# jgsimard/big-dreamer

Hardware: AMD Instinct MI355X
Metric: latent transitions/sec (RSSM + imagination) at batch=50 chunk=50 H=15 (higher is better)
Workload: dtype f32

## Files before the change

### big_dreamer_amd/csrc/observe_cluster.hip

```cpp
#include "bd_cluster.h"

namespace bd {

#ifdef BD_STAMPS
__device__ unsigned long long g_cstamps[64];
#define BD_CSTAMP(slot)                                                                                  \
    do {                                                                                                 \
        if (blockIdx.x == 0 && threadIdx.x == 0 && t == 5) g_cstamps[slot] = __builtin_amdgcn_s_memtime(); \
    } while (0)
#else
#define BD_CSTAMP(slot)
#endif

__global__ __launch_bounds__(kThreads) void observe_cfwd_kernel(bd_observe_fwd_args a_, float* __restrict__ ws, int C,
                                                                int tiles, unsigned spin_limit) {
    extern __shared__ __attribute__((aligned(16))) float smem[];
    BD_KARGS(bd_observe_fwd_args, ap);
#define a (*ap)
    const ScanDims d(a.Be, a.S, a.A, a.Hd);
    const int tile = blockIdx.x / C, c = blockIdx.x - tile * C;
    const int row0 = tile * 16;
    const int F = a.Be + a.S;
    const int nh = d.Kb_h * kFragFloats;
    const int Nb = d.Kb_h;
// ... 394 lines not shown
                    const floatx4* __restrict__ Whz = reinterpret_cast<const floatx4*>(a.wt_hz) + off;
                    const floatx4* __restrict__ Whn = reinterpret_cast<const floatx4*>(a.wt_hn) + off;
                    for (int kb = wave; kb < d.Kb_h; kb += kWaves) {
                        const floatx4 ar = R4[kb * 64], az = Z4[kb * 64], ai = I4[kb * 64], ah = H4[kb * 64];
                        const floatx4 bir = Wir[kb * 64], biz = Wiz[kb * 64], bin = Win[kb * 64];
                        const floatx4 bhr = Whr[kb * 64], bhz = Whz[kb * 64], bhn = Whn[kb * 64];
#pragma unroll
                        for (int j = 0; j < 4; ++j) {
                            DX = mfma16(ar[j], bir[j], DX);
                            DH = mfma16(ar[j], bhr[j], DH);
                            DX = mfma16(az[j], biz[j], DX);
                            DH = mfma16(az[j], bhz[j], DH);
                            DX = mfma16(ai[j], bin[j], DX);
                            DH = mfma16(ah[j], bhn[j], DH);
                        }
                    }
                    floatx4* g = G4 + ((wave * kLocalBlocks + bi) * 2) * 64 + lane;
                    g[0] = DX; g[64] = DH;
                }
            }
        }
        lds_barrier();
        float de_keep[4] = {0.f, 0.f, 0.f, 0.f};
        if (reducer) {
            floatx4 DX = floatx4{0.f, 0.f, 0.f, 0.f}, DH = DX;
            for (int w = 0; w < kWaves; ++w) {
                const floatx4* g = G4 + ((w * kLocalBlocks + wave) * 2) * 64 + lane;
                DX += g[0]; DH += g[64];
            }
            const int col = my_nb * 16 + (lane & 15);
            float* xb = xbuf + (size_t)(epoch & 1) * X.bwd_copy;
#pragma unroll
            for (int r = 0; r < 4; ++r) {
                const int grow = row0 + 4 * (lane >> 4) + r;
                const int off = acc_frag_off(my_nb, lane, r);
                float de = 0.f, carry = 0.f;
                if (grow < a.B && col < a.Be) {
                    de = DX[r] * elu_grad_from_out(svx[r]);
                    carry = dhc[off] + DH[r];
                }
                st_sc1(xb + off, carry);
                st_sc1(xb + nh + off, de);
                de_keep[r] = de;
            }
        }
        BD_CSTAMP(20);
        publish(flags + c, epoch);
        if (reducer) {
            const int col = my_nb * 16 + (lane & 15);
#pragma unroll
            for (int r = 0; r < 4; ++r) {
                const int grow = row0 + 4 * (lane >> 4) + r;
                if (grow < a.B && col < a.Be) a.d_embed_pre[(tb + grow) * a.Be + col] = de_keep[r];
            }
        }
        BD_CSTAMP(21);
        wait_all(flags, C, epoch, err, spin_limit, kErrBwd);
        BD_CSTAMP(22);
        gather_payload(xbuf + (size_t)(epoch & 1) * X.bwd_copy, dhc, 2 * nh);
        lds_barrier();
        BD_KARGS_FRESH(ap);
        BD_CSTAMP(23);
        tile_linear<1>(dE, d.Kb_h, a.wt_embed_s, nullptr, a.S, [&](int, int nb, floatx4 acc) {
            const int col = nb * 16 + (lane & 15);
#pragma unroll
            for (int r = 0; r < 4; ++r) {
                const int row = 4 * (lane >> 4) + r, grow = row0 + row;
                if (col < a.S) {
                    float v = 0.f;
                    if (grow < a.B) v = acc[r] * (a.nonterm ? a.nonterm[tb + grow] : 1.f);
                    ds_plain[row * a.S + col] = v;
                }
            }
        }, scratch);
        lds_barrier();
        BD_CSTAMP(24);
    }
#undef a
}

static int pick_cluster(int B, int Be) {
    const int Nb = cdiv(Be, 16), tiles = cdiv(B, 16);
    int C = tiles * Nb <= 256 ? Nb : cdiv(Nb, kLocalBlocks);
    if (C < 1) C = 1;
    return (C <= kMaxCluster && tiles * C <= 256) ? C : 0;
}

unsigned& cluster_spin_limit() {
    static unsigned v = kSpinLimit;
    return v;
}

}

extern "C" {
using namespace bd;

#ifdef BD_STAMPS
int bd_debug_cstamps(unsigned long long* out64) {
    return hipMemcpyFromSymbol(out64, HIP_SYMBOL(g_cstamps), sizeof(unsigned long long) * 64) == hipSuccess ? 0 : -1;
}
#endif

int bd_observe_cluster_size(int B, int Be) { return pick_cluster(B, Be); }

size_t bd_observe_cluster_ws_floats(int B, int Be) {
    const int tiles = cdiv(B, 16);
    size_t per_tile = ObsClusterWs(cdiv(Be, 16)).per_tile;
    const int C = pick_cluster(B, Be);
    if (C > 0 && kKsCopies * KsBuf(C).total > per_tile) per_tile = kKsCopies * KsBuf(C).total;
    return cluster_ws_header_floats(tiles) + (size_t)tiles * per_tile;
}

size_t bd_observe_cluster_err_offset(int B) { return cluster_ws_flag_floats(cdiv(B, 16)); }

size_t bd_scan_lds_bytes(int kernel, int Be, int S, int D, int C, int A, int Hd, int Cm) {
    const bool cat = kernel >= BD_SCAN_OBSERVE_CAT_FWD && kernel <= BD_SCAN_OBSERVE_CAT_CBWD;
    const bool catc = kernel == BD_SCAN_OBSERVE_CAT_CFWD || kernel == BD_SCAN_OBSERVE_CAT_CBWD;
    if (kernel < BD_SCAN_OBSERVE_FWD || kernel > BD_SCAN_OBSERVE_CAT_CBWD) return fail("bd_scan_lds_bytes: unknown kernel %d", kernel), 0;
    if (Be <= 0 || A <= 0 || Hd <= 0 || (cat ? (D <= 0 || C <= 0) : S <= 0)) return fail("bd_scan_lds_bytes: bad dims"), 0;
    if (catc && (Cm <= 0 || D % Cm != 0)) return fail("bd_scan_lds_bytes: cluster size %d does not divide D=%d", Cm, D), 0;
    const ScanDims d(Be, cat ? 0 : S, A, Hd);
    const int nfm = catc ? D / Cm : D, nbl = nfm * C / 16;
    int total = 0;
    bool ok = false;
#define BD_LAYOUT(id, ...)            \
    case id: {                        \
        const __VA_ARGS__;            \
        total = L.total;              \
        ok = L.vec_ok();              \
    } break
    switch (kernel) {
        BD_LAYOUT(BD_SCAN_OBSERVE_FWD, ObserveFwdLds L(d, S, kObsFwdScratch));
        BD_LAYOUT(BD_SCAN_OBSERVE_BWD, ObserveBwdLds L(d, S, kObsBwdScratch));
        BD_LAYOUT(BD_SCAN_OBSERVE_CFWD, ObserveFwdLds L(d, S, kObsCfwdScratch));
        BD_LAYOUT(BD_SCAN_OBSERVE_CBWD, ObserveBwdLds L(d, S, kObsCbwdScratch));
        BD_LAYOUT(BD_SCAN_OBSERVE_KFWD, KsplitFwdLds L(d, S));
        BD_LAYOUT(BD_SCAN_OBSERVE_KBWD, KsplitBwdLds L(d, S));
        BD_LAYOUT(BD_SCAN_IMAGINE_FWD, ImagineFwdLds L(d, A));
        BD_LAYOUT(BD_SCAN_IMAGINE_BWD, ImagineBwdLds L(d, S));
        BD_LAYOUT(BD_SCAN_OBSERVE_CAT_FWD, CatObserveFwdLds L(d, Be, D, CatFull(D, C), 0));
        BD_LAYOUT(BD_SCAN_OBSERVE_CAT_BWD, CatObserveBwdLds L(d, CatGeo(D, C), 0));
        BD_LAYOUT(BD_SCAN_IMAGINE_CAT_FWD, CatImagineFwdLds L(d, Be, Hd, D, A, CatFull(D, C)));
        BD_LAYOUT(BD_SCAN_IMAGINE_CAT_BWD, CatImagineBwdLds L(d, CatGeo(D, C)));
        BD_LAYOUT(BD_SCAN_OBSERVE_CAT_CFWD, CatObserveFwdLds L(d, Be, D, CatFull(nfm, C), cat_cluster_scratch(nbl, true)));
        BD_LAYOUT(BD_SCAN_OBSERVE_CAT_CBWD, CatObserveBwdLds L(d, CatGeo(nfm, C), cat_cluster_scratch(nbl, false)));
    }
#undef BD_LAYOUT
    if (!ok) return fail("bd_scan_lds_bytes: kernel %d: misaligned LDS layout", kernel), 0;
    return (size_t)total * sizeof(float);
}

int bd_observe_cluster_set_ksplit(int mode) {
    if (mode != -1 && mode != 0) return fail("bd_observe_cluster_set_ksplit: mode %d (expected -1 or 0)", mode);
    ksplit_mode() = mode;
    return 0;
}

int bd_observe_cluster_set_spin_limit(unsigned limit) {
    cluster_spin_limit() = limit ? limit : kSpinLimit;
    return 0;
}

int bd_observe_cluster_status(float* ws, int B, void* stream) {
    unsigned* w = reinterpret_cast<unsigned*>(ws) + bd_observe_cluster_err_offset(B);
    unsigned e = 0;
    if (hipMemcpyAsync(&e, w, sizeof(e), hipMemcpyDeviceToHost, (hipStream_t)stream) != hipSuccess ||
        hipStreamSynchronize((hipStream_t)stream) != hipSuccess)
        return fail("bd_observe_cluster_status: copy failed");
    if (e == 0) return 0;
    if (hipMemsetAsync(w, 0, sizeof(e), (hipStream_t)stream) != hipSuccess) return fail("bd_observe_cluster_status: clear failed");
    return fail("bd_observe_cluster_status: a cluster member timed out waiting for its peers (%s%s scan): results of that "
                "launch are wrong", (e & kErrFwd) ? "forward" : "", (e & kErrBwd) ? ((e & kErrFwd) ? "+backward" : "backward") : "");
}

int bd_observe_forward_cluster(const bd_observe_fwd_args* a, float* ws, size_t ws_floats, void* stream) {
    BD_REQUIRE(a && ws && a->T > 0 && a->B > 0 && a->Be > 0 && a->S > 0 && a->A > 0 && a->Hd > 0,
               "bd_observe_forward_cluster: bad arguments");
    BD_REQUIRE(a->w_embed_s && a->w_embed_a && a->b_embed && a->w_ir && a->w_iz && a->w_in && a->w_hr && a->w_hz &&
                   a->w_hn && a->b_ih && a->b_hh && a->w_q1h && a->b_q1 && a->w_q2m && a->w_q2s && a->b_q2 &&
                   a->init_belief && a->init_state && a->actions && a->pre_emb && a->eps_post && a->feat &&
                   a->post_mean && a->post_std, "bd_observe_forward_cluster: missing pointers");
    BD_REQUIRE(a->S <= kHeadMaxN, "bd_observe_forward_cluster: state width above %d", kHeadMaxN);
    const int C = pick_cluster(a->B, a->Be);
    BD_REQUIRE(C > 0, "bd_observe_forward_cluster: B=%d, Be=%d do not fit the cluster variant", a->B, a->Be);
    const int tiles = cdiv(a->B, 16);
    BD_REQUIRE(ws_floats >= bd_observe_cluster_ws_floats(a->B, a->Be), "bd_observe_forward_cluster: workspace too small");
    const ScanDims d(a->Be, a->S, a->A, a->Hd);
    const ObserveFwdLds L(d, a->S, kObsCfwdScratch);
    BD_REQUIRE(L.vec_ok(), "bd_observe_forward_cluster: misaligned LDS layout");
    const size_t lds = (size_t)L.total * sizeof(float);
    BD_REQUIRE(lds <= (size_t)kMaxLds, "bd_observe_forward_cluster: needs %zu B of LDS", lds);
    if (ksplit_ok(a->Be, a->S, a->A, a->Hd, C))
        return launch_observe_kfwd(a, ws, C, tiles, (hipStream_t)stream);
    if (allow_big_lds(observe_cfwd_kernel)) return -1;
    const size_t dyn = launch_lds(observe_cfwd_kernel, lds, "bd_observe_forward_cluster");
    if (!dyn) return -1;
    if (hipMemsetAsync(ws, 0, cluster_ws_flag_floats(tiles) * sizeof(float), (hipStream_t)stream) != hipSuccess)
        return fail("bd_observe_forward_cluster: memset failed");
    hipLaunchKernelGGL(observe_cfwd_kernel, dim3(tiles * C), dim3(kThreads), dyn, (hipStream_t)stream, *a, ws, C, tiles,
                       cluster_spin_limit());
    BD_CHECK_LAUNCH("bd_observe_forward_cluster");
    return 0;
}

int bd_observe_backward_cluster(const bd_observe_bwd_args* a, float* ws, size_t ws_floats, void* stream) {
    BD_REQUIRE(a && ws && a->T > 0 && a->B > 0 && a->Be > 0 && a->S > 0 && a->A > 0 && a->Hd > 0,
               "bd_observe_backward_cluster: bad arguments");
    BD_REQUIRE(a->wt_embed_s && a->wt_ir && a->wt_iz && a->wt_in && a->wt_hr && a->wt_hz && a->wt_hn && a->wt_q1h &&
                   a->wt_q2m && a->wt_q2s && a->init_belief && a->eps_post && a->feat && a->post_std && a->sv_x &&
                   a->sv_gates && a->sv_q && a->dfeat && a->d_embed_pre && a->d_gi && a->d_gh && a->d_q1_pre && a->d_q2_out,
               "bd_observe_backward_cluster: missing pointers");
    const int C = pick_cluster(a->B, a->Be);
    BD_REQUIRE(C > 0, "bd_observe_backward_cluster: B=%d, Be=%d do not fit the cluster variant", a->B, a->Be);
    const int tiles = cdiv(a->B, 16);
    BD_REQUIRE(ws_floats >= bd_observe_cluster_ws_floats(a->B, a->Be), "bd_observe_backward_cluster: workspace too small");
    const ScanDims d(a->Be, a->S, a->A, a->Hd);
    const ObserveBwdLds L(d, a->S, kObsCbwdScratch);
    BD_REQUIRE(L.vec_ok(), "bd_observe_backward_cluster: misaligned LDS layout");
    const size_t lds = (size_t)L.total * sizeof(float);
    BD_REQUIRE(lds <= (size_t)kMaxLds, "bd_observe_backward_cluster: needs %zu B of LDS", lds);
    if (ksplit_ok(a->Be, a->S, a->A, a->Hd, C)) return launch_observe_kbwd(a, ws, C, tiles, (hipStream_t)stream);
    if (allow_big_lds(observe_cbwd_kernel)) return -1;
    const size_t dyn = launch_lds(observe_cbwd_kernel, lds, "bd_observe_backward_cluster");
    if (!dyn) return -1;
    if (hipMemsetAsync(ws, 0, cluster_ws_flag_floats(tiles) * sizeof(float), (hipStream_t)stream) != hipSuccess)
        return fail("bd_observe_backward_cluster: memset failed");
    hipLaunchKernelGGL(observe_cbwd_kernel, dim3(tiles * C), dim3(kThreads), dyn, (hipStream_t)stream, *a, ws, C, tiles,
                       cluster_spin_limit());
    BD_CHECK_LAUNCH("bd_observe_backward_cluster");
    return 0;
}

}
```

### big_dreamer_amd/csrc/observe_ksplit.hip

```cpp
#include "bd_cluster.h"

namespace bd {

#ifdef BD_STAMPS
__device__ unsigned long long g_kstamps[64];
#define BD_KSTAMP(slot)                                                                                  \
    do {                                                                                                 \
        if (blockIdx.x == 0 && threadIdx.x == 0 && t == 5) g_kstamps[slot] = __builtin_amdgcn_s_memtime(); \
    } while (0)
#else
#define BD_KSTAMP(slot)
#endif

constexpr int kKsMaxS = 4;
constexpr int kKsMaxA = 2;

__device__ __forceinline__ void ks_store4(float* p, floatx4 v) {
    asm volatile("s_nop 7\n\ts_nop 3\n\tglobal_store_dwordx4 %0, %1, off sc1\n\ts_nop 1" ::"v"(p), "v"(v) : "memory");
}
__device__ __forceinline__ floatx4 ks_load4(const float* p) {
    const unsigned long long lo = ld_sc1_u64(p), hi = ld_sc1_u64(p + 2);
    return floatx4{__uint_as_float((unsigned)lo), __uint_as_float((unsigned)(lo >> 32)), __uint_as_float((unsigned)hi),
                   __uint_as_float((unsigned)(hi >> 32))};
}
// ... 195 lines not shown
        float* hx = xb + kb_.g;
        BD_KSTAMP(0);
        BD_KARGS_FRESH(ap);
        BD_KSTAMP(1);
        {
            const floatx4* __restrict__ S4 = reinterpret_cast<const floatx4*>(sf) + lane;
            const floatx4* __restrict__ A4 = reinterpret_cast<const floatx4*>(af) + lane;
#pragma unroll
            for (int i = 0; i < 2; ++i) {
                const int nbo = wave + kWaves * i;
                if (nbo < Kb_h) {
                    floatx4 acc = be4x[i];
#pragma unroll
                    for (int kb = 0; kb < kKsMaxS; ++kb)
                        if (kb < Kb_s) acc = mfmaT(we_s[i][kb], S4[kb * 64], acc);
#pragma unroll
                    for (int kb = 0; kb < kKsMaxA; ++kb)
                        if (kb < Kb_a) acc = mfmaT(we_a[i][kb], A4[kb * 64], acc);
                    floatx4 x4;
                    const int col0 = nbo * 16 + 4 * (lane >> 4);
#pragma unroll
                    for (int j = 0; j < 4; ++j) x4[j] = (rok && col0 + j < a.Be) ? elu(acc[j]) : 0.f;
                    XF4[nbo * 64 + lane] = x4;
                    if (nbo == c && rok && a.sv_x) ks_put4(a.sv_x + (tb + grow) * a.Be + fcol0, x4, nbe);
                }
            }
        }
        lds_barrier();
        BD_KSTAMP(2);
        BD_KARGS_FRESH(ap);
        {
            floatx4 R = z4, Z = z4, NI = z4, NH = z4;
#pragma unroll
            for (int i = 0; i < 2; ++i) {
                const int kb = wave + kWaves * i;
                if (kb < Kb_h) {
                    const floatx4 xk = XF4[kb * 64 + lane], hk = HF4[kb * 64 + lane];
                    R = mfmaT(wg[i][0], xk, R); Z = mfmaT(wg[i][1], xk, Z); NI = mfmaT(wg[i][2], xk, NI);
                    R = mfmaT(wg[i][3], hk, R); Z = mfmaT(wg[i][4], hk, Z); NH = mfmaT(wg[i][5], hk, NH);
                }
            }
            GP4[(wave * 4 + 0) * 64 + lane] = R; GP4[(wave * 4 + 1) * 64 + lane] = Z;
            GP4[(wave * 4 + 2) * 64 + lane] = NI; GP4[(wave * 4 + 3) * 64 + lane] = NH;
        }
        lds_barrier();
        BD_KSTAMP(3);
        BD_KSTAMP(4);
        {
            const int g = wave & 3, half = wave >> 2;
            floatx4 s4 = z4;
#pragma unroll
            for (int w = 0; w < 4; ++w) s4 += GP4[((half * 4 + w) * 4 + g) * 64 + lane];
            RED4[wave * 64 + lane] = s4;
        }
        lds_barrier();
        {
            const floatx4 R = RED4[0 * 64 + lane] + RED4[4 * 64 + lane] + br4, Z = RED4[1 * 64 + lane] + RED4[5 * 64 + lane] + bz4;
            const floatx4 NI = RED4[2 * 64 + lane] + RED4[6 * 64 + lane] + bni4, NH = RED4[3 * 64 + lane] + RED4[7 * 64 + lane] + bnh4;
            floatx4 rr4, zz4, nn4;
#pragma unroll
            for (int i = 0; i < 4; ++i) {
                rr4[i] = sigmoidf(R[i]);
                zz4[i] = sigmoidf(Z[i]);
                nn4[i] = tanh_act(NI[i] + rr4[i] * NH[i]);
                h4[i] = (rok && i < nbe) ? (1.f - zz4[i]) * nn4[i] + zz4[i] * h4[i] : 0.f;
            }
            if (wave == 0) {
                ks_store4(hx + (size_t)c * 256 + lane * 4, h4);
                if (rok) {
                    ks_put4(a.feat + (tb + grow) * F + fcol0, h4, nbe);
                    if (a.sv_gates) {
                        float* gg = a.sv_gates + (tb + grow) * 4 * a.Be + fcol0;
                        ks_put4(gg, rr4, nbe); ks_put4(gg + a.Be, zz4, nbe); ks_put4(gg + 2 * a.Be, nn4, nbe); ks_put4(gg + 3 * a.Be, NH, nbe);
                    }
                }
            }
        }
        BD_KSTAMP(5);
        BD_KARGS_FRESH(ap);
        const float n_nt = load_nt(t + 1, tid), n_ac = load_ac(t + 1, tid);
        const floatx4 pre4 = rok ? ks_row4(a.pre_emb + (tb + grow) * a.Hd + fcol0, nhd) : z4;
        float eps = 0.f;
        {
            const int row = tid / a.S, col = tid - row * a.S;
            if (tid < 16 * a.S && row0 + row < a.B) eps = a.eps_post[(tb + row0 + row) * a.S + col];
        }
#pragma unroll
        for (int i = 0; i < 2; ++i) {
            const int nbo = wave + kWaves * i;
            if (nbo < Kb_hd) ks_emit(xb + kb_.q + (size_t)(nbo * C + c) * kKsImg, lane, mfmaT(wq[i], h4, z4));
        }
        BD_KSTAMP(6);
        ks_handoff(flags, c, C, (unsigned)(3 * t + 2), err, spin_limit, kErrFwd);
        BD_KSTAMP(7);
        REDB[wave * 64 + lane] = c < Kb_hd ? ks_reduce(xb + kb_.q + (size_t)(c * C) * kKsImg, kKsImg, wave, kWaves, C, lane) : z4;
#pragma unroll
        for (int i = 0; i < 2; ++i) {
            const int nbo = wave + kWaves * i;
            if (nbo < Kb_h) HF4[nbo * 64 + lane] = ks_load4(hx + (size_t)nbo * 256 + lane * 4);
        }
        lds_barrier();
        floatx4 q4 = bq4 + pre4;
        for (int w = 0; w < kWaves; ++w) q4 += REDB[w * 64 + lane];
#pragma unroll
        for (int i = 0; i < 4; ++i) q4[i] = (rok && i < nhd) ? elu(q4[i]) : 0.f;
        if (wave == 0 && rok && a.sv_q) ks_put4(a.sv_q + (tb + grow) * a.Hd + fcol0, q4, nhd);
        BD_KSTAMP(8);
        BD_KARGS_FRESH(ap);
        if (has_pair) ks_emit(xb + kb_.s + (size_t)(c * 8 + pair) * kKsImg, lane, mfmaT(wh, q4, z4));
        BD_KSTAMP(9);
        ks_handoff(flags, c, C, (unsigned)(3 * t + 3), err, spin_limit, kErrFwd);
        BD_KSTAMP(10);
        BD_KARGS_FRESH(ap);
        if (sums_pair) {
            floatx4 v = ks_reduce(xb + kb_.s + (size_t)pair * kKsImg, (size_t)8 * kKsImg, part, nparts, C, lane);
            if (part == 0) v += bh4;
            float* pl = plain + (size_t)part * 2 * 16 * Np;
#pragma unroll
            for (int i = 0; i < 4; ++i) pl[pair_raw * 16 * Np + frow * Np + pair_nb * 16 + 4 * (lane >> 4) + i] = v[i];
        }
        lds_barrier();
        if (tid < 16 * a.S) {
            const int e = tid;
            const int row = e / a.S, col = e - row * a.S;
            const int gr = row0 + row;
            float st = 0.f;
            if (gr < a.B) {
                float Mn = plain[row * Np + col], Rw = plain[16 * Np + row * Np + col];
                for (int pt = 1; pt < nparts; ++pt) {
                    Mn += plain[pt * 2 * 16 * Np + row * Np + col];
                    Rw += plain[pt * 2 * 16 * Np + 16 * Np + row * Np + col];
                }
                const float ee = eps;
                const float sd = softplusf(Rw) + a.min_std;
                st = Mn + sd * ee;
                if (lead) {
                    const size_t ix = (tb + gr) * a.S + col;
                    a.post_mean[ix] = Mn;
                    a.post_std[ix] = sd;
                    a.feat[(tb + gr) * F + a.Be + col] = st;
                }
            }
            const float mv = st * n_nt;
            sf[frag_idx(row, col)] = mv;
            if (lead && a.sv_s && t + 1 < a.T && gr < a.B) a.sv_s[(tb + a.B + gr) * a.S + col] = mv;
        }
        if (tid < 16 * Kb_a * 16) af[frag_idx(tid / (Kb_a * 16), tid % (Kb_a * 16))] = n_ac;
        lds_barrier();
        BD_KSTAMP(11);
    }
#undef a
}

__global__ __launch_bounds__(kThreads) void observe_kbwd_kernel(bd_observe_bwd_args a_, float* __restrict__ ws, int C, int tiles,
                                                                unsigned spin_limit) {
    extern __shared__ __attribute__((aligned(16))) float smem[];
    BD_KARGS(bd_observe_bwd_args, ap);
#define a (*ap)
    const ScanDims d(a.Be, a.S, a.A, a.Hd);
    const int Kb_h = d.Kb_h, Kb_s = d.Kb_s, Kb_hd = d.Kb_hd;
    const int tile = blockIdx.x / C, c = blockIdx.x - tile * C;
    const int row0 = tile * 16, F = a.Be + a.S;
    const int lane = threadIdx.x & 63;
    const int wave = __builtin_amdgcn_readfirstlane((int)(threadIdx.x >> 6));
    const KsplitBwdLds L(d, a.S);
    float* dM = smem + L.dM;
    float* dRaw = smem + L.dRaw;
    float* ds_plain = smem + L.ds_plain;
    const int nparts = L.nparts;
    const int dsp_stride = L.dsp_stride;
    float* red = smem + L.red;

    unsigned* flags = reinterpret_cast<unsigned*>(ws) + tile * kMaxCluster;
    unsigned* err = reinterpret_cast<unsigned*>(ws) + tiles * kMaxCluster;
    const KsBuf kb_(C);
    float* xbase = ws + cluster_ws_header_floats(tiles) + (size_t)tile * kKsCopies * kb_.total;

    floatx4 w2m[kKsMaxS], w2s[kKsMaxS];
#pragma unroll
    for (int kb = 0; kb < kKsMaxS; ++kb) {
        w2m[kb] = ks_frag(a.wt_q2m, c, Kb_s, kb, lane, kb < Kb_s && c < Kb_hd);
        w2s[kb] = ks_frag(a.wt_q2s, c, Kb_s, kb, lane, kb < Kb_s && c < Kb_hd);
    }
    floatx4 w1[2], wg[2][6];
#pragma unroll
    for (int i = 0; i < 2; ++i) {
        const int nbo = wave + kWaves * i;
        const bool ok = nbo < Kb_h;
        w1[i] = ks_frag(a.wt_q1h, nbo, Kb_hd, c, lane, ok && c < Kb_hd);
        wg[i][0] = ks_frag(a.wt_ir, nbo, Kb_h, c, lane, ok); wg[i][1] = ks_frag(a.wt_iz, nbo, Kb_h, c, lane, ok);
        wg[i][2] = ks_frag(a.wt_in, nbo, Kb_h, c, lane, ok); wg[i][3] = ks_frag(a.wt_hr, nbo, Kb_h, c, lane, ok);
        wg[i][4] = ks_frag(a.wt_hz, nbo, Kb_h, c, lane, ok); wg[i][5] = ks_frag(a.wt_hn, nbo, Kb_h, c, lane, ok);
    }
    const int sblk = wave % Kb_s, spart = wave / Kb_s;
    floatx4 wes = ks_frag(a.wt_embed_s, sblk, Kb_h, c, lane, spart == 0);
    const int frow = lane & 15, fcol0 = c * 16 + 4 * (lane >> 4);
    const int grow = row0 + frow;
    const int nbe = a.Be - fcol0 < 0 ? 0 : (a.Be - fcol0 < 4 ? a.Be - fcol0 : 4);
    const int nhd = a.Hd - fcol0 < 0 ? 0 : (a.Hd - fcol0 < 4 ? a.Hd - fcol0 : 4);
    const bool rok = grow < a.B;

    for (int i = threadIdx.x; i < nparts * dsp_stride; i += blockDim.x) ds_plain[i] = 0.f;
    lds_barrier();

    KS_SETTLE_BEGIN();
    ks_settle(w2m); ks_settle(w2s); ks_settle(w1); ks_settle(wg[0]); ks_settle(wg[1]);
    ks_settle(wes);
    const bool lead = (c == 0);
    floatx4* __restrict__ RED4 = reinterpret_cast<floatx4*>(red);
    floatx4* __restrict__ REDB = RED4 + kWaves * 64;
    const floatx4 z4 = floatx4{0.f, 0.f, 0.f, 0.f};
    floatx4 dhc4 = z4;
    unsigned epoch = 0;

    struct B1v { float dfs, dpm, eps, dps, pstd; };
    struct Svv { floatx4 svq4, svx4, gr4, gz4, gn4, gh4, hp4, dft4; };
    auto load_b1 = [&](int t, int i) {
        B1v v{0.f, 0.f, 0.f, 0.f, 0.f};
        const int r = i / (Kb_s * 16), k = i - r * (Kb_s * 16);
        const int gr = row0 + r;
        if (i < 16 * Kb_s * 16 && gr < a.B && k < a.S) {
            const size_t tb = (size_t)t * a.B, idx = (tb + gr) * a.S + k;
            v.dfs = a.dfeat[(tb + gr) * F + a.Be + k];
            v.dpm = a.dpost_mean ? a.dpost_mean[idx] : 0.f;
            v.eps = a.eps_post[idx];
            v.dps = a.dpost_std ? a.dpost_std[idx] : 0.f;
            v.pstd = a.post_std[idx];
        }
        return v;
    };
    auto load_sv = [&](int t) {
        Svv v;
        v.svq4 = floatx4{1.f, 1.f, 1.f, 1.f};
        v.svx4 = v.svq4;
        v.gr4 = v.gz4 = v.gn4 = v.gh4 = v.hp4 = v.dft4 = z4;
        if (rok) {
            const size_t tb = (size_t)t * a.B;
            v.svq4 = ks_row4(a.sv_q + (tb + grow) * a.Hd + fcol0, nhd);
            v.svx4 = ks_row4(a.sv_x + (tb + grow) * a.Be + fcol0, nbe);
            const float* gg = a.sv_gates + (tb + grow) * 4 * a.Be + fcol0;
            v.gr4 = ks_row4(gg, nbe); v.gz4 = ks_row4(gg + a.Be, nbe); v.gn4 = ks_row4(gg + 2 * a.Be, nbe); v.gh4 = ks_row4(gg + 3 * a.Be, nbe);
            v.hp4 = t > 0 ? ks_row4(a.feat + (tb - a.B + grow) * F + fcol0, nbe) : ks_row4(a.init_belief + (size_t)grow * a.Be + fcol0, nbe);
            v.dft4 = ks_row4(a.dfeat + (tb + grow) * F + fcol0, nbe);
        }
        return v;
    };
    B1v nb1{0.f, 0.f, 0.f, 0.f, 0.f};
    Svv nsv{z4, z4, z4, z4, z4, z4, z4, z4};
    nb1 = load_b1(a.T - 1, (int)threadIdx.x);
    nsv = load_sv(a.T - 1);

    for (int t = a.T - 1; t >= 0; --t) {
        const size_t tb = (size_t)t * a.B;
        const int tid = bd_tid();
        float* xb = xbase + (size_t)(t & 1) * kb_.total;
        BD_KSTAMP(16);
        BD_KARGS_FRESH(ap);
        const B1v cb1 = nb1;
        const Svv sv = nsv;
        if (t > 0) {
            nb1 = load_b1(t - 1, tid);
            nsv = load_sv(t - 1);
        }
        if (tid < 16 * Kb_s * 16) {
            const int i = tid;
            const int r = i / (Kb_s * 16), k = i - r * (Kb_s * 16);
            const int gr = row0 + r;
            float dm = 0.f, dr = 0.f;
            if (gr < a.B && k < a.S) {
                const B1v v = cb1;
                float dst = v.dfs;
                for (int pt = 0; pt < nparts; ++pt) dst += ds_plain[pt * dsp_stride + r * a.S + k];
                dm = dst + v.dpm;
                const float dsd = dst * v.eps + v.dps;
                dr = dsd * one_minus_exp_neg(v.pstd - a.min_std);
                if (lead) {
                    a.d_q2_out[(tb + gr) * 2 * a.S + k] = dm;
                    a.d_q2_out[(tb + gr) * 2 * a.S + a.S + k] = dr;
                }
            }
            dM[frag_idx(r, k)] = dm;
            dRaw[frag_idx(r, k)] = dr;
        }
        const floatx4 svq4 = sv.svq4, svx4 = sv.svx4, gr4 = sv.gr4, gz4 = sv.gz4, gn4 = sv.gn4, gh4 = sv.gh4, hp4 = sv.hp4, dft4 = sv.dft4;
        lds_barrier();
        BD_KSTAMP(17);
        floatx4 dq4;
        {
            floatx4 acc = z4;
            const floatx4* __restrict__ M4 = reinterpret_cast<const floatx4*>(dM) + lane;
            const floatx4* __restrict__ R4 = reinterpret_cast<const floatx4*>(dRaw) + lane;
#pragma unroll
            for (int kb = 0; kb < kKsMaxS; ++kb)
                if (kb < Kb_s) {
                    acc = mfmaT(w2m[kb], M4[kb * 64], acc);
                    acc = mfmaT(w2s[kb], R4[kb * 64], acc);
                }
#pragma unroll
            for (int i = 0; i < 4; ++i) dq4[i] = (rok && i < nhd) ? acc[i] * elu_grad_from_out(svq4[i]) : 0.f;
            if (wave == 0 && rok) ks_put4(a.d_q1_pre + (tb + grow) * a.Hd + fcol0, dq4, nhd);
        }
        BD_KSTAMP(18);
        BD_KARGS_FRESH(ap);
        ++epoch;
#pragma unroll
        for (int i = 0; i < 2; ++i) {
            const int nbo = wave + kWaves * i;
            if (nbo < Kb_h) ks_emit(xb + kb_.q + (size_t)(nbo * C + c) * kKsImg, lane, mfmaT(w1[i], dq4, z4));
        }
        BD_KSTAMP(19);
        ks_handoff(flags, c, C, epoch, err, spin_limit, kErrBwd);
        BD_KSTAMP(20);
        RED4[wave * 64 + lane] = ks_reduce(xb + kb_.q + (size_t)(c * C) * kKsImg, kKsImg, wave, kWaves, C, lane);
        lds_barrier();
        floatx4 vr4, vz4, vni4, vnh4, carry4;
        {
            floatx4 dh4 = dhc4 + dft4;
            for (int w = 0; w < kWaves; ++w) dh4 += RED4[w * 64 + lane];
#pragma unroll
            for (int i = 0; i < 4; ++i) {
                const bool ok = rok && i < nbe;
                const float dh = ok ? dh4[i] : 0.f;
                const float rr = gr4[i], zz = gz4[i], nn = gn4[i], hn = gh4[i];
                const float dn = dh * (1.f - zz);
                const float dz = dh * (hp4[i] - nn);
                vni4[i] = dn * (1.f - nn * nn);
                vnh4[i] = vni4[i] * rr;
                vr4[i] = vni4[i] * hn * rr * (1.f - rr);
                vz4[i] = dz * zz * (1.f - zz);
                carry4[i] = dh * zz;
            }
            if (wave == 0 && rok) {
                float* gi = a.d_gi + (tb + grow) * 3 * a.Be + fcol0;
                float* ghh = a.d_gh + (tb + grow) * 3 * a.Be + fcol0;
                ks_put4(gi, vr4, nbe); ks_put4(gi + a.Be, vz4, nbe); ks_put4(gi + 2 * a.Be, vni4, nbe);
                ks_put4(ghh, vr4, nbe); ks_put4(ghh + a.Be, vz4, nbe); ks_put4(ghh + 2 * a.Be, vnh4, nbe);
            }
        }
        BD_KSTAMP(21);
        BD_KARGS_FRESH(ap);
        ++epoch;
#pragma unroll
        for (int i = 0; i < 2; ++i) {
            const int nbo = wave + kWaves * i;
            if (nbo < Kb_h) {
                floatx4 DX = mfmaT(wg[i][0], vr4, z4), DH = mfmaT(wg[i][3], vr4, z4);
                DX = mfmaT(wg[i][1], vz4, DX); DH = mfmaT(wg[i][4], vz4, DH);
                DX = mfmaT(wg[i][2], vni4, DX); DH = mfmaT(wg[i][5], vnh4, DH);
                float* dst = xb + kb_.g + ((size_t)(nbo * C + c) * 2) * kKsImg;
                ks_emit(dst, lane, DX); ks_emit(dst + kKsImg, lane, DH);
            }
        }
        BD_KSTAMP(22);
        ks_handoff(flags, c, C, epoch, err, spin_limit, kErrBwd);
        BD_KSTAMP(23);
        {
            const int g = wave & 1, quarter = wave >> 1;
            REDB[wave * 64 + lane] = ks_reduce(xb + kb_.g + ((size_t)(c * C) * 2 + g) * kKsImg, (size_t)2 * kKsImg, quarter, 4, C, lane);
        }
        lds_barrier();
        floatx4 de4;
        {
            floatx4 DX = z4, DH = z4;
            for (int qd = 0; qd < 4; ++qd) { DX += REDB[(2 * qd) * 64 + lane]; DH += REDB[(2 * qd + 1) * 64 + lane]; }
#pragma unroll
            for (int i = 0; i < 4; ++i) {
                const bool ok = rok && i < nbe;
                de4[i] = ok ? DX[i] * elu_grad_from_out(svx4[i]) : 0.f;
                dhc4[i] = ok ? carry4[i] + DH[i] : 0.f;
            }
            if (wave == 0 && rok) ks_put4(a.d_embed_pre + (tb + grow) * a.Be + fcol0, de4, nbe);
        }
        BD_KSTAMP(24);
        BD_KARGS_FRESH(ap);
        ++epoch;
        if (spart == 0) ks_emit(xb + kb_.s + (size_t)(c * 8 + sblk) * kKsImg, lane, mfmaT(wes, de4, z4));
        BD_KSTAMP(25);
        ks_handoff(flags, c, C, epoch, err, spin_limit, kErrBwd);
        BD_KSTAMP(26);
        BD_KARGS_FRESH(ap);
        if (spart < nparts) {
            const floatx4 v = ks_reduce(xb + kb_.s + (size_t)sblk * kKsImg, (size_t)8 * kKsImg, spart, nparts, C, lane);
            const float mk = rok ? (a.nonterm ? a.nonterm[tb + grow] : 1.f) : 0.f;
#pragma unroll
            for (int i = 0; i < 4; ++i) {
                const int col = sblk * 16 + 4 * (lane >> 4) + i;
                if (col < a.S) ds_plain[spart * dsp_stride + frow * a.S + col] = v[i] * mk;
            }
        }
        lds_barrier();
        BD_KSTAMP(27);
    }
#undef a
}

int& ksplit_mode() {
    static int m = -1;
    return m;
}

bool ksplit_ok(int Be, int S, int A, int Hd, int C) {
    if (ksplit_mode() == 0) return false;
    return C == cdiv(Be, 16) && C <= 2 * kWaves && cdiv(Hd, 16) <= C && cdiv(S, 16) <= kKsMaxS && cdiv(A, 16) <= kKsMaxA &&
           S <= kHeadMaxN && 16 * S <= kThreads && 2 * cdiv(S, 16) <= kWaves;
}

static int ks_reset(float* ws, int tiles, hipStream_t stream, const char* who) {
    if (hipMemsetAsync(ws, 0, cluster_ws_flag_floats(tiles) * sizeof(float), stream) != hipSuccess) return fail("%s: memset failed", who);
    return 0;
}

int launch_observe_kfwd(const bd_observe_fwd_args* a, float* ws, int C, int tiles, hipStream_t stream) {
    if (allow_big_lds(observe_kfwd_ns_kernel)) return -1;
    const KsplitFwdLds L(ScanDims(a->Be, a->S, a->A, a->Hd), a->S);
    BD_REQUIRE(L.vec_ok(), "bd_observe_forward_cluster: misaligned LDS layout");
    const size_t dyn = launch_lds(observe_kfwd_ns_kernel, (size_t)L.total * sizeof(float), "bd_observe_forward_cluster");
    if (!dyn) return -1;
    if (ks_reset(ws, tiles, stream, "bd_observe_forward_cluster")) return -1;
    hipLaunchKernelGGL(observe_kfwd_ns_kernel, dim3(tiles * C), dim3(kThreads), dyn, stream, *a, ws, C, tiles, cluster_spin_limit());
    BD_CHECK_LAUNCH("bd_observe_forward_cluster");
    return 0;
}
int launch_observe_kbwd(const bd_observe_bwd_args* a, float* ws, int C, int tiles, hipStream_t stream) {
    if (allow_big_lds(observe_kbwd_kernel)) return -1;
    const KsplitBwdLds L(ScanDims(a->Be, a->S, a->A, a->Hd), a->S);
    BD_REQUIRE(L.vec_ok(), "bd_observe_backward_cluster: misaligned LDS layout");
    const size_t dyn = launch_lds(observe_kbwd_kernel, (size_t)L.total * sizeof(float), "bd_observe_backward_cluster");
    if (!dyn) return -1;
    if (ks_reset(ws, tiles, stream, "bd_observe_backward_cluster")) return -1;
    hipLaunchKernelGGL(observe_kbwd_kernel, dim3(tiles * C), dim3(kThreads), dyn, stream, *a, ws, C, tiles, cluster_spin_limit());
    BD_CHECK_LAUNCH("bd_observe_backward_cluster");
    return 0;
}

}

#ifdef BD_STAMPS
extern "C" int bd_debug_kstamps(unsigned long long* out64) {
    return hipMemcpyFromSymbol(out64, HIP_SYMBOL(bd::g_kstamps), sizeof(unsigned long long) * 64) == hipSuccess ? 0 : -1;
}
#endif
```

Before: 13.94 million.

## Gather full dq1 per block to drop one cross-block handoff in k-split backward

Adds a GATHER variant of the k-split observe backward kernel. Each block now redundantly computes every dq1 column block itself from locally held dM/dRaw, so the first exchange/handoff/reduce through global memory is no longer needed. The second exchange now emits raw de4 instead of pre-multiplied partials, and the reduction applies the embed weights after gathering. This removes one inter-block spin barrier per timestep at the cost of more redundant MFMA work, more register-resident weight fragments, and a tighter S limit for the k-split path. It is on by default, with the old path kept under mode -3.

New measurement: 14.06 million (median of 6 runs). No clear change (+0.8%).

```diff
diff --git a/big_dreamer_amd/csrc/observe_cluster.hip b/big_dreamer_amd/csrc/observe_cluster.hip
--- a/big_dreamer_amd/csrc/observe_cluster.hip
+++ b/big_dreamer_amd/csrc/observe_cluster.hip
@@ -570,7 +570,7 @@
 }
 
 int bd_observe_cluster_set_ksplit(int mode) {
-    if (mode != -1 && mode != 0) return fail("bd_observe_cluster_set_ksplit: mode %d (expected -1 or 0)", mode);
+    if (mode != -1 && mode != 0 && mode != -3) return fail("bd_observe_cluster_set_ksplit: mode %d (expected -1, 0 or -3)", mode);
     ksplit_mode() = mode;
     return 0;
 }
diff --git a/big_dreamer_amd/csrc/observe_ksplit.hip b/big_dreamer_amd/csrc/observe_ksplit.hip
--- a/big_dreamer_amd/csrc/observe_ksplit.hip
+++ b/big_dreamer_amd/csrc/observe_ksplit.hip
@@ -371,6 +371,9 @@
 #undef a
 }
 
+constexpr int kKsGatherS = 2;
+constexpr int kKsGatherFrags = 4;
+template <bool GATHER>
 __global__ __launch_bounds__(kThreads) void observe_kbwd_kernel(bd_observe_bwd_args a_, float* __restrict__ ws, int C, int tiles,
                                                                 unsigned spin_limit) {
     extern __shared__ __attribute__((aligned(16))) float smem[];
@@ -398,21 +401,40 @@
     floatx4 w2m[kKsMaxS], w2s[kKsMaxS];
 #pragma unroll
     for (int kb = 0; kb < kKsMaxS; ++kb) {
-        w2m[kb] = ks_frag(a.wt_q2m, c, Kb_s, kb, lane, kb < Kb_s && c < Kb_hd);
-        w2s[kb] = ks_frag(a.wt_q2s, c, Kb_s, kb, lane, kb < Kb_s && c < Kb_hd);
+        if constexpr (GATHER) {
+            const int j = wave + kWaves * (kb / kKsGatherS), k = kb % kKsGatherS;
+            w2m[kb] = ks_frag(a.wt_q2m, j, Kb_s, k, lane, k < Kb_s && j < Kb_hd);
+            w2s[kb] = ks_frag(a.wt_q2s, j, Kb_s, k, lane, k < Kb_s && j < Kb_hd);
+        } else {
+            w2m[kb] = ks_frag(a.wt_q2m, c, Kb_s, kb, lane, kb < Kb_s && c < Kb_hd);
+            w2s[kb] = ks_frag(a.wt_q2s, c, Kb_s, kb, lane, kb < Kb_s && c < Kb_hd);
+        }
     }
     floatx4 w1[2], wg[2][6];
 #pragma unroll
     for (int i = 0; i < 2; ++i) {
         const int nbo = wave + kWaves * i;
         const bool ok = nbo < Kb_h;
-        w1[i] = ks_frag(a.wt_q1h, nbo, Kb_hd, c, lane, ok && c < Kb_hd);
+        if constexpr (GATHER) w1[i] = ks_frag(a.wt_q1h, c, Kb_hd, nbo, lane, nbo < Kb_hd);
+        else w1[i] = ks_frag(a.wt_q1h, nbo, Kb_hd, c, lane, ok && c < Kb_hd);
         wg[i][0] = ks_frag(a.wt_ir, nbo, Kb_h, c, lane, ok); wg[i][1] = ks_frag(a.wt_iz, nbo, Kb_h, c, lane, ok);
         wg[i][2] = ks_frag(a.wt_in, nbo, Kb_h, c, lane, ok); wg[i][3] = ks_frag(a.wt_hr, nbo, Kb_h, c, lane, ok);
         wg[i][4] = ks_frag(a.wt_hz, nbo, Kb_h, c, lane, ok); wg[i][5] = ks_frag(a.wt_hn, nbo, Kb_h, c, lane, ok);
     }
     const int sblk = wave % Kb_s, spart = wave / Kb_s;
-    floatx4 wes = ks_frag(a.wt_embed_s, sblk, Kb_h, c, lane, spart == 0);
+    floatx4 wes = ks_frag(a.wt_embed_s, sblk, Kb_h, c, lane, !GATHER && spart == 0);
+    floatx4 wesg[kKsGatherFrags];
+#pragma unroll
+    for (int i = 0; i < kKsGatherFrags; ++i) {
+        const int m = spart + nparts * i;
+        wesg[i] = ks_frag(a.wt_embed_s, sblk, Kb_h, m < C ? m : 0, lane, GATHER && spart < nparts && m < C);
+    }
+    int qcol[2], nq[2];
+#pragma unroll
+    for (int i = 0; i < 2; ++i) {
+        qcol[i] = (wave + kWaves * i) * 16 + 4 * (lane >> 4);
+        nq[i] = a.Hd - qcol[i] < 0 ? 0 : (a.Hd - qcol[i] < 4 ? a.Hd - qcol[i] : 4);
+    }
     const int frow = lane & 15, fcol0 = c * 16 + 4 * (lane >> 4);
     const int grow = row0 + frow;
     const int nbe = a.Be - fcol0 < 0 ? 0 : (a.Be - fcol0 < 4 ? a.Be - fcol0 : 4);
@@ -424,7 +446,8 @@
 
     KS_SETTLE_BEGIN();
     ks_settle(w2m); ks_settle(w2s); ks_settle(w1); ks_settle(wg[0]); ks_settle(wg[1]);
-    ks_settle(wes);
+    if constexpr (GATHER) ks_settle(wesg);
+    else ks_settle(wes);
     const bool lead = (c == 0);
     floatx4* __restrict__ RED4 = reinterpret_cast<floatx4*>(red);
     floatx4* __restrict__ REDB = RED4 + kWaves * 64;
@@ -433,7 +456,7 @@
     unsigned epoch = 0;
 
     struct B1v { float dfs, dpm, eps, dps, pstd; };
-    struct Svv { floatx4 svq4, svx4, gr4, gz4, gn4, gh4, hp4, dft4; };
+    struct Svv { floatx4 svq4, svqb4, svx4, gr4, gz4, gn4, gh4, hp4, dft4; };
     auto load_b1 = [&](int t, int i) {
         B1v v{0.f, 0.f, 0.f, 0.f, 0.f};
         const int r = i / (Kb_s * 16), k = i - r * (Kb_s * 16);
@@ -451,11 +474,16 @@
     auto load_sv = [&](int t) {
         Svv v;
         v.svq4 = floatx4{1.f, 1.f, 1.f, 1.f};
-        v.svx4 = v.svq4;
+        v.svx4 = v.svqb4 = v.svq4;
         v.gr4 = v.gz4 = v.gn4 = v.gh4 = v.hp4 = v.dft4 = z4;
         if (rok) {
             const size_t tb = (size_t)t * a.B;
-            v.svq4 = ks_row4(a.sv_q + (tb + grow) * a.Hd + fcol0, nhd);
+            if constexpr (GATHER) {
+                if (nq[0] > 0) v.svq4 = ks_row4(a.sv_q + (tb + grow) * a.Hd + qcol[0], nq[0]);
+                if (nq[1] > 0) v.svqb4 = ks_row4(a.sv_q + (tb + grow) * a.Hd + qcol[1], nq[1]);
+            } else {
+                v.svq4 = ks_row4(a.sv_q + (tb + grow) * a.Hd + fcol0, nhd);
+            }
             v.svx4 = ks_row4(a.sv_x + (tb + grow) * a.Be + fcol0, nbe);
             const float* gg = a.sv_gates + (tb + grow) * 4 * a.Be + fcol0;
             v.gr4 = ks_row4(gg, nbe); v.gz4 = ks_row4(gg + a.Be, nbe); v.gn4 = ks_row4(gg + 2 * a.Be, nbe); v.gh4 = ks_row4(gg + 3 * a.Be, nbe);
@@ -465,7 +493,7 @@
         return v;
     };
     B1v nb1{0.f, 0.f, 0.f, 0.f, 0.f};
-    Svv nsv{z4, z4, z4, z4, z4, z4, z4, z4};
+    Svv nsv{z4, z4, z4, z4, z4, z4, z4, z4, z4};
     nb1 = load_b1(a.T - 1, (int)threadIdx.x);
     nsv = load_sv(a.T - 1);
 
@@ -504,33 +532,61 @@
         const floatx4 svq4 = sv.svq4, svx4 = sv.svx4, gr4 = sv.gr4, gz4 = sv.gz4, gn4 = sv.gn4, gh4 = sv.gh4, hp4 = sv.hp4, dft4 = sv.dft4;
         lds_barrier();
         BD_KSTAMP(17);
-        floatx4 dq4;
-        {
-            floatx4 acc = z4;
+        if constexpr (GATHER) {
             const floatx4* __restrict__ M4 = reinterpret_cast<const floatx4*>(dM) + lane;
             const floatx4* __restrict__ R4 = reinterpret_cast<const floatx4*>(dRaw) + lane;
-#pragma unroll
-            for (int kb = 0; kb < kKsMaxS; ++kb)
-                if (kb < Kb_s) {
-                    acc = mfmaT(w2m[kb], M4[kb * 64], acc);
-                    acc = mfmaT(w2s[kb], R4[kb * 64], acc);
+            floatx4 part4 = z4;
+#pragma unroll
+            for (int i = 0; i < 2; ++i) {
+                const int j = wave + kWaves * i;
+                if (j < Kb_hd) {
+                    floatx4 acc = z4, dq4;
+#pragma unroll
+                    for (int kb = 0; kb < kKsGatherS; ++kb)
+                        if (kb < Kb_s) {
+                            acc = mfmaT(w2m[i * kKsGatherS + kb], M4[kb * 64], acc);
+                            acc = mfmaT(w2s[i * kKsGatherS + kb], R4[kb * 64], acc);
+                        }
+                    const floatx4 q4 = i ? sv.svqb4 : sv.svq4;
+#pragma unroll
+                    for (int k = 0; k < 4; ++k) dq4[k] = (rok && k < nq[i]) ? acc[k] * elu_grad_from_out(q4[k]) : 0.f;
+                    if (j == c && rok) ks_put4(a.d_q1_pre + (tb + grow) * a.Hd + fcol0, dq4, nhd);
+                    part4 += mfmaT(w1[i], dq4, z4);
                 }
-#pragma unroll
-            for (int i = 0; i < 4; ++i) dq4[i] = (rok && i < nhd) ? acc[i] * elu_grad_from_out(svq4[i]) : 0.f;
-            if (wave == 0 && rok) ks_put4(a.d_q1_pre + (tb + grow) * a.Hd + fcol0, dq4, nhd);
-        }
-        BD_KSTAMP(18);
-        BD_KARGS_FRESH(ap);
-        ++epoch;
-#pragma unroll
-        for (int i = 0; i < 2; ++i) {
-            const int nbo = wave + kWaves * i;
-            if (nbo < Kb_h) ks_emit(xb + kb_.q + (size_t)(nbo * C + c) * kKsImg, lane, mfmaT(w1[i], dq4, z4));
-        }
-        BD_KSTAMP(19);
-        ks_handoff(flags, c, C, epoch, err, spin_limit, kErrBwd);
-        BD_KSTAMP(20);
-        RED4[wave * 64 + lane] = ks_reduce(xb + kb_.q + (size_t)(c * C) * kKsImg, kKsImg, wave, kWaves, C, lane);
+            }
+            BD_KSTAMP(18);
+            RED4[wave * 64 + lane] = part4;
+            BD_KSTAMP(19);
+            BD_KSTAMP(20);
+        } else {
+            floatx4 dq4;
+            {
+                floatx4 acc = z4;
+                const floatx4* __restrict__ M4 = reinterpret_cast<const floatx4*>(dM) + lane;
+                const floatx4* __restrict__ R4 = reinterpret_cast<const floatx4*>(dRaw) + lane;
+#pragma unroll
+                for (int kb = 0; kb < kKsMaxS; ++kb)
+                    if (kb < Kb_s) {
+                        acc = mfmaT(w2m[kb], M4[kb * 64], acc);
+                        acc = mfmaT(w2s[kb], R4[kb * 64], acc);
+                    }
+#pragma unroll
+                for (int i = 0; i < 4; ++i) dq4[i] = (rok && i < nhd) ? acc[i] * elu_grad_from_out(svq4[i]) : 0.f;
+                if (wave == 0 && rok) ks_put4(a.d_q1_pre + (tb + grow) * a.Hd + fcol0, dq4, nhd);
+            }
+            BD_KSTAMP(18);
+            BD_KARGS_FRESH(ap);
+            ++epoch;
+#pragma unroll
+            for (int i = 0; i < 2; ++i) {
+                const int nbo = wave + kWaves * i;
+                if (nbo < Kb_h) ks_emit(xb + kb_.q + (size_t)(nbo * C + c) * kKsImg, lane, mfmaT(w1[i], dq4, z4));
+            }
+            BD_KSTAMP(19);
+            ks_handoff(flags, c, C, epoch, err, spin_limit, kErrBwd);
+            BD_KSTAMP(20);
+            RED4[wave * 64 + lane] = ks_reduce(xb + kb_.q + (size_t)(c * C) * kKsImg, kKsImg, wave, kWaves, C, lane);
+        }
         lds_barrier();
         floatx4 vr4, vz4, vni4, vnh4, carry4;
         {
@@ -593,13 +649,31 @@
         BD_KSTAMP(24);
         BD_KARGS_FRESH(ap);
         ++epoch;
-        if (spart == 0) ks_emit(xb + kb_.s + (size_t)(c * 8 + sblk) * kKsImg, lane, mfmaT(wes, de4, z4));
+        if constexpr (GATHER) {
+            if (wave == 0) ks_emit(xb + kb_.s + (size_t)c * kKsImg, lane, de4);
+        } else {
+            if (spart == 0) ks_emit(xb + kb_.s + (size_t)(c * 8 + sblk) * kKsImg, lane, mfmaT(wes, de4, z4));
+        }
         BD_KSTAMP(25);
         ks_handoff(flags, c, C, epoch, err, spin_limit, kErrBwd);
         BD_KSTAMP(26);
         BD_KARGS_FRESH(ap);
         if (spart < nparts) {
-            const floatx4 v = ks_reduce(xb + kb_.s + (size_t)sblk * kKsImg, (size_t)8 * kKsImg, spart, nparts, C, lane);
+            floatx4 v;
+            if constexpr (GATHER) {
+                floatx4 de[kKsGatherFrags];
+#pragma unroll
+                for (int i = 0; i < kKsGatherFrags; ++i) {
+                    const int m = spart + nparts * i;
+                    de[i] = z4;
+                    if (m < C) de[i] = ks_load4(xb + kb_.s + (size_t)m * kKsImg + lane * 4);
+                }
+                v = z4;
+#pragma unroll
+                for (int i = 0; i < kKsGatherFrags; ++i) v += mfmaT(wesg[i], de[i], z4);
+            } else {
+                v = ks_reduce(xb + kb_.s + (size_t)sblk * kKsImg, (size_t)8 * kKsImg, spart, nparts, C, lane);
+            }
             const float mk = rok ? (a.nonterm ? a.nonterm[tb + grow] : 1.f) : 0.f;
 #pragma unroll
             for (int i = 0; i < 4; ++i) {
@@ -621,7 +695,7 @@
 bool ksplit_ok(int Be, int S, int A, int Hd, int C) {
     if (ksplit_mode() == 0) return false;
     return C == cdiv(Be, 16) && C <= 2 * kWaves && cdiv(Hd, 16) <= C && cdiv(S, 16) <= kKsMaxS && cdiv(A, 16) <= kKsMaxA &&
-           S <= kHeadMaxN && 16 * S <= kThreads && 2 * cdiv(S, 16) <= kWaves;
+           S <= kHeadMaxN && 16 * S <= kThreads && 2 * cdiv(S, 16) <= kWaves && cdiv(S, 16) <= kKsGatherS;
 }
 
 static int ks_reset(float* ws, int tiles, hipStream_t stream, const char* who) {
@@ -640,16 +714,21 @@
     BD_CHECK_LAUNCH("bd_observe_forward_cluster");
     return 0;
 }
-int launch_observe_kbwd(const bd_observe_bwd_args* a, float* ws, int C, int tiles, hipStream_t stream) {
-    if (allow_big_lds(observe_kbwd_kernel)) return -1;
+template <bool GATHER>
+static int launch_kbwd(const bd_observe_bwd_args* a, float* ws, int C, int tiles, hipStream_t stream) {
+    if (allow_big_lds(observe_kbwd_kernel<GATHER>)) return -1;
     const KsplitBwdLds L(ScanDims(a->Be, a->S, a->A, a->Hd), a->S);
     BD_REQUIRE(L.vec_ok(), "bd_observe_backward_cluster: misaligned LDS layout");
-    const size_t dyn = launch_lds(observe_kbwd_kernel, (size_t)L.total * sizeof(float), "bd_observe_backward_cluster");
+    const size_t dyn = launch_lds(observe_kbwd_kernel<GATHER>, (size_t)L.total * sizeof(float), "bd_observe_backward_cluster");
     if (!dyn) return -1;
     if (ks_reset(ws, tiles, stream, "bd_observe_backward_cluster")) return -1;
-    hipLaunchKernelGGL(observe_kbwd_kernel, dim3(tiles * C), dim3(kThreads), dyn, stream, *a, ws, C, tiles, cluster_spin_limit());
+    hipLaunchKernelGGL(observe_kbwd_kernel<GATHER>, dim3(tiles * C), dim3(kThreads), dyn, stream, *a, ws, C, tiles,
+                       cluster_spin_limit());
     BD_CHECK_LAUNCH("bd_observe_backward_cluster");
     return 0;
+}
+int launch_observe_kbwd(const bd_observe_bwd_args* a, float* ws, int C, int tiles, hipStream_t stream) {
+    return ksplit_mode() == -3 ? launch_kbwd<false>(a, ws, C, tiles, stream) : launch_kbwd<true>(a, ws, C, tiles, stream);
 }
 
 }
```
